# TobiaMarcucci/warm-start-hybrid-mpc

Measured on AMD Instinct MI355X. Metric: QP subproblems/sec, cart-pole-with-walls N=20 synthetic frontier, higher is better.
Workload: dtype f64

## Files before the change

warm-start-hybrid-mpc_amd/csrc/hmpc_device.h:

```cpp
#ifndef HMPC_DEVICE_H
#define HMPC_DEVICE_H

#include <stdint.h>

#include "hmpc.h"

struct SparseStage {
    int m, mg;
    const int *rptr, *rcol;
    const double *rval;
    const int *cptr, *crow;
    const double *cval;
    const int *gptr, *grow;
    const double *gval;
    const double *h;
    const double *scale;
};

#define HMPC_KC_STRIDE 16

struct DevProb {
    int nx, nu, nub, nuc, nz, T, nc, ncL, nT, mreg, Toff, M, Mpad, n, ne, nq, nr, nqT, n_primal, n_dual;
    unsigned mreg_magic;
    int nnz0, nng0;
    SparseStage reg;
    const double *Creg;
    const double *ccv;
    const int *cci;
    int kcol;
    int ngram;
    const double *F_raw, *G_raw, *h_raw, *hT_raw;
    const double *shift_Mmu, *shift_Mrho, *shift_V;
    int *work_counter;
    unsigned *check_flag;
    double *fac_ws;
    int fac_stride;
    int ring;
    int nd, ndp, ns;
    const double *Cdn;
    const int *drow;
    const int *rinfo;
    const double *sval;
    const int *sptr, *srow;
    const int *nrow;
    unsigned nd_magic, nn_magic;
    int split_lds;
    int static_rows;
    const double *Ct, *ht, *sct;
    const double *A, *B, *P, *PT, *Q, *R, *QT;
    const int *ei, *ej;
    double cs;
    double tol, tol_inf;
    int max_iter, lazy, refine;
    int dbg;
    int polish;
    int polish_l1;
    double ptol;
};

struct DevOut {
    double *obj, *dual_obj;
    int32_t *status, *iters;
    double *primal, *dual;
};

struct DevWarm {
    const double *primal, *dual;
    const int32_t *index;
    int32_t *pend;
    int32_t second;
};

static inline size_t hmpc_lds_bytes(const DevProb &p, int kc, int big)
{
    const size_t n = p.n, T = p.T, nx = p.nx, nu = p.nu, nz = p.nz, nub = p.nub, M = p.M;
    size_t d = 0, i = 0, b = 0;
    const size_t nxs = nx * (nx + 1) / 2, lms = nx * nu + nu * (nu - 1) / 2;
    const size_t dir = n + (T + 1) * nx + T * nub, fscr = nz * nz + (kc > 0 ? nz * nz : nx * nz);
    d += dir;
    d += M;
    d += T * nu + (big ? 0 : T * lms + (T + 1) * nxs);
    d += n + T * nx + (T + 1) * nx + n + (T + 1) * nx;
    d += dir + (dir > fscr ? dir : fscr);
    d += (nx + 3) / 4 * 4 + nz + 40;
    d += nx;
    if (big) {
        const size_t nur = (nu + 3) / 4 * 4, nup = (nu + 1 + 3) / 4 * 4, lrows = nz + 1 > nx + nur ? nz + 1 : nx + nur;
        d += ((nx + 1 + 3) / 4 * 4) * lrows + nz * nz + nx * nx;
        d += 2 * (size_t)p.ring * lrows * nup + lms;
    } else {
        d += nx * nz + nz * nz + nx * nx;
    }
    i += 2 + T * nub + 2 * (size_t)p.ne;
    if (!big) {
        i += (p.ne + 1) + p.nng0;
        d += p.mreg + p.nng0;
    }
    if (big) {
    } else if (kc > 0) {
        d += nz * (size_t)kc;
        b += (nz * (size_t)kc + 3) / 4 * 4;
    } else {
        d += 2 * (size_t)p.nnz0;
        i += (p.mreg + 1) + p.nnz0 + (nz + 1) + p.nnz0;
    }
    if (kc == 0 && p.split_lds) {
        d += (size_t)p.ndp * nz + p.mreg;
        i += (size_t)p.ndp + p.mreg + (nz + 1) + p.ns + (p.mreg - p.nd);
    }
    return d * sizeof(double) + i * sizeof(int) + b;
}

#endif
```

warm-start-hybrid-mpc_amd/csrc/hmpc_kernel.hip:

```cpp
#include <hip/hip_runtime.h>
#include <math.h>
#include <stdint.h>
#include <type_traits>

#include "hmpc_device.h"

#define WAVE 64
#define HMPC_REFINE_FROM_IT 12
#define HMPC_POLISH_RHO 1e5
#define HMPC_POLISH_RHO2 1e7
#define HMPC_POLISH_DELTA 1e-10
#define HMPC_RHO_OF(level) ((level) == 1 ? HMPC_POLISH_RHO2 : HMPC_POLISH_RHO)
#define HMPC_POLISH_ITERS 5
#define HMPC_POLISH_ROUNDS 6
#define HMPC_POLISH_ROUNDS_LAST 10
#define HMPC_ESC_MAX 2
#define HMPC_ESC_ITERS 6
#define HMPC_ESC_ENABLED(D) true
#define HMPC_LAM0_ROW 1
#ifndef HMPC_STABLE_DEN
#define HMPC_STABLE_DEN 1
#endif
#ifndef HMPC_PAIR
#define HMPC_PAIR 1
#endif
#ifndef HMPC_NARROW_PANEL
#define HMPC_NARROW_PANEL 1
#endif
#define HMPC_POLISH_ATTEMPTS 3
#define HMPC_RETRY (-1)
#define HMPC_POLISH_ROUNDS_WARM 3
#ifndef HMPC_POLISH_ROUNDS_OWN
#define HMPC_POLISH_ROUNDS_OWN 8
#endif
#define HMPC_POLISH_WARM_BMOVE 0.5
#define HMPC_POLISH_WARM_VMAX 1e-2
#ifndef HMPC_KERNEL_ATTR
#define HMPC_KERNEL_ATTR
#endif
#define DEV __device__ __forceinline__
#ifdef HMPC_NO_FENCE
#define HMPC_FENCE() do { } while (0)
#else
#define HMPC_FENCE() __builtin_amdgcn_sched_barrier(0)
#endif

#ifdef HMPC_STAMPS
#define DBG_SKIP(bit) (p.dbg & (1 << (bit)))
#define STAMP(k) do { long long now_ = clock64(); tacc[k] += now_ - tlast; tlast = clock64(); } while (0)
#define FSTAMP(k) do { long long now_ = clock64(); facc[k] += now_ - flast; flast = clock64(); } while (0)
#define FSTAMP_DECL long long flast = clock64()
static __device__ long long facc_dump[16];
#define FSTAMP_ARGS , long long *facc
#define FSTAMP_PASS , facc
#else
#define DBG_SKIP(bit) false
#define STAMP(k) do { } while (0)
#define FSTAMP(k) do { } while (0)
#define FSTAMP_DECL do { } while (0)
#define FSTAMP_ARGS
#define FSTAMP_PASS
#endif

DEV void lds_barrier()
{
    asm volatile("s_waitcnt lgkmcnt(0)\n\ts_barrier" ::: "memory");
}

DEV double wave_sum(double v)
{
#pragma unroll
    for (int o = 32; o > 0; o >>= 1) v += __shfl_xor(v, o);
    return v;
}
DEV double wave_max(double v)
{
#pragma unroll
    for (int o = 32; o > 0; o >>= 1) v = fmax(v, __shfl_xor(v, o));
    return v;
}
DEV double wave_min(double v)
{
#pragma unroll
    for (int o = 32; o > 0; o >>= 1) v = fmin(v, __shfl_xor(v, o));
    return v;
}

template <class D, int N>
DEV void block_reduce(double (&v)[N], const int (&op)[N], __attribute__((address_space(3))) double *red, int tid)
{
#pragma unroll
    for (int i = 0; i < N; i++) v[i] = op[i] == 0 ? wave_sum(v[i]) : op[i] == 1 ? wave_max(v[i]) : wave_min(v[i]);
    if constexpr (D::kNW > 1) {
        if ((tid & 63) == 0) {
#pragma unroll
            for (int i = 0; i < N; i++) red[(tid >> 6) * N + i] = v[i];
        }
        __syncthreads();
#pragma unroll
        for (int i = 0; i < N; i++) {
            double a = red[i];
#pragma unroll
            for (int w = 1; w < D::kNW; w++) {
                const double b = red[w * N + i];
                a = op[i] == 0 ? a + b : op[i] == 1 ? fmax(a, b) : fmin(a, b);
            }
            v[i] = a;
        }
        __syncthreads();
    }
}
template <class D> DEV double block_sum(double x, __attribute__((address_space(3))) double *red, int tid)
{
    double v[1] = {x};
    const int op[1] = {0};
    block_reduce<D, 1>(v, op, red, tid);
    return v[0];
}
template <class D> DEV double block_max(double x, __attribute__((address_space(3))) double *red, int tid)
{
    double v[1] = {x};
    const int op[1] = {1};
    block_reduce<D, 1>(v, op, red, tid);
    return v[0];
}
template <class D> DEV double block_min(double x, __attribute__((address_space(3))) double *red, int tid)
{
    double v[1] = {x};
    const int op[1] = {2};
    block_reduce<D, 1>(v, op, red, tid);
    return v[0];
}

DEV double bcast(double v, int src)
{
    const int lo = __builtin_amdgcn_readlane(__double2loint(v), src);
    const int hi = __builtin_amdgcn_readlane(__double2hiint(v), src);
    return __hiloint2double(hi, lo);
}

template <class D> DEV double bcast16(double v, int src)
{
    if constexpr (!D::kDpp) return bcast(v, src);
    const long x = __builtin_bit_cast(long, v);
    long r;
    switch (src) {
#define HMPC_DPP_CASE(n) case n: r = __builtin_amdgcn_update_dpp((long)0, x, 0x150 + n, 0xf, 0xf, false); break;
        HMPC_DPP_CASE(0) HMPC_DPP_CASE(1) HMPC_DPP_CASE(2) HMPC_DPP_CASE(3) HMPC_DPP_CASE(4) HMPC_DPP_CASE(5) HMPC_DPP_CASE(6) HMPC_DPP_CASE(7)
        HMPC_DPP_CASE(8) HMPC_DPP_CASE(9) HMPC_DPP_CASE(10) HMPC_DPP_CASE(11) HMPC_DPP_CASE(12) HMPC_DPP_CASE(13) HMPC_DPP_CASE(14)
#undef HMPC_DPP_CASE
    default: r = __builtin_amdgcn_update_dpp((long)0, x, 0x150 + 15, 0xf, 0xf, false); break;
    }
    return __builtin_bit_cast(double, r);
}

DEV double frcp(double b)
{
    double r = __builtin_amdgcn_rcp(b);
    r = fma(fma(-b, r, 1.0), r, r);
    r = fma(fma(-b, r, 1.0), r, r);
    return r;
}

typedef __attribute__((address_space(3))) double ldsd;
typedef __attribute__((address_space(3))) int ldsi;
typedef __attribute__((address_space(3))) unsigned char ldsb;

template <class IP, class DP>
struct Lists {
    IP rptr, rcol, cptr, crow, gptr, grow;
    DP rval, cval, gval, h;
};
typedef Lists<const ldsi *, const ldsd *> ListsL;
typedef Lists<const int *, const double *> ListsG;

struct Lds {
    ldsd *w, *lam, *nuf;
// ... 889 lines not shown
        }
#pragma unroll
        for (int qp = 0; qp < MQ; qp += 2) {
            if (stage && have[qp] && have[qp + 1] && (nx & 3) == 0) {
                const int i0 = trow[qp] + c0, ic0 = i0 < nz ? i0 : nz - 1, jc0 = colq[qp] < nz ? colq[qp] : nz - 1;
                const int i1 = trow[qp + 1] + c0, ic1 = i1 < nz ? i1 : nz - 1, jc1 = colq[qp + 1] < nz ? colq[qp + 1] : nz - 1;
                mfma_d4 acc0 = {gq[qp][0], gq[qp][1], gq[qp][2], gq[qp][3]}, acc1 = {gq[qp + 1][0], gq[qp + 1][1], gq[qp + 1][2], gq[qp + 1][3]};
                mfma_pair_k4<5>(wl, nx, [&](int, int k) { return S.AB[k * AB_STRIDE + ic0]; }, [&](int k, int) { return S.PA[k * nz + jc0]; },
                                [&](int, int k) { return S.AB[k * AB_STRIDE + ic1]; }, [&](int k, int) { return S.PA[k * nz + jc1]; }, acc0, acc1);
#pragma unroll
                for (int r = 0; r < 4; r++) { m[qp][r] = acc0[r]; m[qp + 1][r] = acc1[r]; }
            }
        }
#pragma unroll
        for (int qq = 0; qq < MQ; qq++) {
            if (stage && have[qq]) {
                if (!(have[qq & ~1] && have[qq | 1] && (nx & 3) == 0)) {
                const int i = trow[qq] + c0, ic = i < nz ? i : nz - 1, jc = colq[qq] < nz ? colq[qq] : nz - 1;
                mfma_d4 acc = {gq[qq][0], gq[qq][1], gq[qq][2], gq[qq][3]};
                if ((nx & 3) == 0)
                    acc = mfma_tile_k4<5>(wl, nx, [&](int, int k) { return S.AB[k * AB_STRIDE + ic]; }, [&](int k, int) { return S.PA[k * nz + jc]; }, acc);
                else
                    acc = mfma_tile_batched<5>(wl, nx, [&](int, int k) { return S.AB[k * AB_STRIDE + ic]; },
                                               [&](int k, int) { return S.PA[k * nz + jc]; }, acc);
#pragma unroll
                for (int r = 0; r < 4; r++) m[qq][r] = acc[r];
                }
                if (tcol[qq] + 15 >= nx) {
#pragma unroll
                    for (int r = 0; r < 4; r++) {
                        const int row = row0[qq] + 4 * r, col = colq[qq];
                        ldsd *w = (row < nz && col < nz) ? Mf + row * nz + col : dump;
                        *w = m[qq][r];
                    }
                }
                if (trow[qq] != tcol[qq] && trow[qq] + 15 >= nx) {
#pragma unroll
                    for (int r = 0; r < 4; r++) {
                        const int row = row0[qq] + 4 * r, col = colq[qq];
                        ldsd *w = (row < nz && col < nz) ? Mf + col * nz + row : dump;
                        *w = m[qq][r];
                    }
                }
            }
        }
        if (stage) lds_barrier();
        FSTAMP(1);
        if (!tilew) {
          if (stage) {
            const int i = lane, ic = i < nz ? i : 0, b0 = nx + nuc;
            const int fxv = i < nub ? fx[i < nub ? i : 0] : -1;
            const unsigned long long fm1 = __ballot(fxv >= 0), fone = __ballot(fxv == 1);
            unsigned fixmask = (unsigned)(fm1 << nuc);
            if (i < nz) {
                double g = 0;
                for (int b = 0; b < nub; b++)
                    if ((fone >> b) & 1ull) g += Mf[i * nz + b0 + b];
                S.g[t * nz + i] = g;
            }
            const bool rowfixed = i >= nx && i < nz && ((fixmask >> (i - nx)) & 1u);
            auto panel = [&](auto nc_, int ncols) {
                constexpr int NC = decltype(nc_)::value;
                double a[NC];
#pragma unroll
                for (int k = 0; k < NC; k++) {
                    const double x = Mf[ic * nz + nx + (k < ncols ? k : 0)];
                    const bool pres = rowfixed || ((fixmask >> k) & 1u);
                    a[k] = (k < ncols && i < nz) ? (pres ? (i == nx + k ? 1.0 : 0.0) : x) : 0.0;
                }
                int nuo = __builtin_amdgcn_readfirstlane(ncols);
                unsigned fmask = __builtin_amdgcn_readfirstlane(fixmask);
#pragma unroll
                for (int j = 0; j < NC; j++) {
                    asm volatile("" : "+s"(nuo), "+s"(fmask));
                    if (j < nuo) {
                        if (i < nz) Mf[i * nz + nx + j] = a[j];
                        if ((fmask >> j) & 1u) {
                            if (lane == 0) S.dinv[t * nu + j] = 1.0;
                        } else {
                            const double d = bcast(a[j], nx + j);
                            if (!(d > 0.0)) bad = 1;
                            double rinv = __builtin_amdgcn_rcp(d);
                            rinv = rinv * (2.0 - d * rinv);
                            const bool trailing = i < nx || (i > nx + j && i < nz);
                            const double mval = a[j] * rinv, meff = trailing ? mval : 0.0;
#pragma unroll
                            for (int k = j + 1; k < NC; k++) a[k] -= meff * bcast(a[k], nx + j);
                            if (trailing) Lw[i < nx ? LM_X(nx, nu, i, j) : LM_U(nx, nu, i - nx, j)] = mval;
                            if (lane == 0) S.dinv[t * nu + j] = rinv;
                        }
                    }
                }
            };
            constexpr int NUMC = 8;
            if (HMPC_NARROW_PANEL && nub > 0 && nuc <= NUMC && __popcll(fm1) == nub) {
                panel(std::integral_constant<int, NUMC>(), nuc);
                if (lane < nub) S.dinv[t * nu + nuc + lane] = 1.0;
            } else {
                panel(std::integral_constant<int, NUM>(), nu);
            }
            if (bad && lane == 0) S.flag[0] = 1;
          }
        } else if (t > 0) {
            gram(t - 1);
        }
        if (!stage) continue;
        lds_barrier();
        FSTAMP(3);
#pragma unroll
        for (int qq = 0; qq < MQ; qq++) {
            if (have[qq] && trow[qq] < nx && tcol[qq] < nx) {
                const int i = trow[qq] + c0, ixc = i < nx ? i : nx - 1, k = colq[qq], kc = k < nx ? k : nx - 1;
                mfma_d4 acc = {m[qq][0], m[qq][1], m[qq][2], m[qq][3]};
                acc = mfma_tile_batched<4>(wl, nu, [&](int, int j) { return -Lw[LM_X(nx, nu, ixc, j)]; },
                                           [&](int j, int) { return Mf[kc * nz + nx + j]; }, acc);
#pragma unroll
                for (int r = 0; r < 4; r++) {
                    const int row = row0[qq] + 4 * r, col = colq[qq];
                    if (row < nx && col <= row) {
                        const double v = acc[r];
                        Mf[row * nz + col] = v;
                        Mf[col * nz + row] = v;
                        fac_pr<D>(S)[t * nxs + sym(row, col)] = v;
                    }
                }
            }
        }
        if constexpr (D::kBig)
            for (int e = lane; e < lms; e += D::kNT) Lm[e] = Lw[e];
        lds_barrier();
        FSTAMP(4);
    }
    __syncthreads();
    return (bad || S.flag[0]) ? -1 : 0;
}

template <class D> DEV int factor_reg(const DevProb &p, const Lds &S, int lane FSTAMP_ARGS)
{
    constexpr int NX = D::kNX, NU = D::kNU, NUB = D::kNUB, NUC = NU - NUB, NZ = NX + NU, NE = NZ * (NZ + 1) / 2;
    static_assert(NZ <= 16, "the register recursions broadcast inside one row of 16 lanes");
    constexpr int NXS = NX * (NX + 1) / 2, LMS = LM_STAGE(NX, NU), KG = D::kKC, GH = KG / 2;
    const int T = p.T;
    FSTAMP_DECL;
    LANE_OPAQUE(lane);
    if (lane == 0) S.flag[0] = 0;
    if (D::kNW == 1 || lane < WAVE) {
        const int ng = p.ngram;
        const bool has = lane < ng;
        const int ge = has ? lane : 0;
        const int gi = S.ei[ge], gj = S.ej[ge];
        const int gp0 = S.L0.gptr[ge], glen = has ? S.L0.gptr[ge + 1] - gp0 : 0;
        const double pij = S.P[gi * NZ + gj];
        ldsd *TG = S.Mm + NZ * NZ;
        for (int q = ng + lane; q < NE; q += WAVE) {
            const int i = S.ei[q], j = S.ej[q];
            const double a = S.P[i * NZ + j];
            S.Mm[i * NZ + j] = a;
            S.Mm[j * NZ + i] = a;
        }
        if (S.term_on) {
            const ldsd *Dt = S.e + p.Toff;
            if (p.nT == 0) {
                for (int q = lane; q < NZ * NZ; q += WAVE) TG[q] = 0.0;
            }
            for (int r0 = 0; r0 < p.nT; r0 += WAVE) {
                const int row = r0 + lane;
                const bool ok = row < p.nT;
                const int rc = ok ? row : 0;
                const double dr = ok ? Dt[rc] : 0.0;
                const double *c = p.Ct + (size_t)rc * NZ;
                double cr[NZ];
#pragma unroll
                for (int j = 0; j < NZ; j++) cr[j] = c[j];
#pragma unroll
                for (int i = 0; i < NZ; i++) {
#pragma unroll
                    for (int j = 0; j <= i; j++) {
                        const double a = wave_sum(cr[i] * cr[j] * dr);
                        if (lane == 0) {
                            const double v = (r0 ? TG[i * NZ + j] : 0.0) + a;
                            TG[i * NZ + j] = v;
                            TG[j * NZ + i] = v;
                        }
                    }
                }
            }
        }
        double ABc[NX], pn[NX];
#pragma unroll
        for (int l = 0; l < NX; l++) ABc[l] = lane < NZ ? S.AB[l * NZ + lane] : 0.0;
#pragma unroll
        for (int i = 0; i < NX; i++) pn[i] = lane < NX ? S.PT[i * NX + lane] : 0.0;
        if (lane < NX) {
#pragma unroll
            for (int i = 0; i < NX; i++)
                if (i >= lane) S.Pr[T * NXS + sym(i, lane)] = pn[i];
        }
        int bad = 0;
        for (int t = T - 1; t >= 0; t--) {
            const ldsi *fx = S.fix + t * NUB;
            ldsd *Lm = S.Lm + t * LMS;
            int fxv[NUB];
#pragma unroll
            for (int b = 0; b < NUB; b++) fxv[b] = fx[b];
            double g0 = pij, g1 = 0.0;
            {
                const ldsd *Dt = S.e + t * p.mreg;
#pragma unroll
                for (int hb = 0; hb < KG; hb += GH) {
                    int idx[GH];
                    double gv[GH], dv[GH];
#pragma unroll
                    for (int q = 0; q < GH; q++) {
                        const int qq = gp0 + (hb + q < glen ? hb + q : 0);
                        idx[q] = S.L0.grow[qq];
                        gv[q] = S.L0.gval[qq];
                    }
                    HMPC_FENCE();
#pragma unroll
                    for (int q = 0; q < GH; q++) { HMPC_CHK(idx[q] >= 0 && idx[q] < p.mreg, 2); dv[q] = Dt[idx[q]]; }
                    HMPC_FENCE();
#pragma unroll
                    for (int q = 0; q < GH; q++) {
                        const double term = hb + q < glen ? gv[q] * dv[q] : 0.0;
                        if (q & 1) g1 += term;
                        else g0 += term;
                    }
                }
            }
            if (has) {
                S.Mm[gi * NZ + gj] = g0 + g1;
                S.Mm[gj * NZ + gi] = g0 + g1;
            }
            if (ng > WAVE) {
                const bool has2 = WAVE + lane < ng;
                const int ge2 = has2 ? WAVE + lane : 0;
                const int gi2 = S.ei[ge2], gj2 = S.ej[ge2];
                const int gq0 = S.L0.gptr[ge2], glen2 = has2 ? S.L0.gptr[ge2 + 1] - gq0 : 0;
                const ldsd *Dt = S.e + t * p.mreg;
                double h0 = S.P[gi2 * NZ + gj2], h1 = 0.0;
#pragma unroll
                for (int q = 0; q < KG; q++) {
                    const int qq = gq0 + (q < glen2 ? q : 0);
                    const double term = q < glen2 ? S.L0.gval[qq] * Dt[S.L0.grow[qq]] : 0.0;
                    if (q & 1) h1 += term;
                    else h0 += term;
                }
                if (has2) {
                    S.Mm[gi2 * NZ + gj2] = h0 + h1;
                    S.Mm[gj2 * NZ + gi2] = h0 + h1;
                }
            }
            double y[NX];
#pragma unroll
            for (int i = 0; i < NX; i++) {
                double a = 0.0;
#pragma unroll
                for (int l = 0; l < NX; l++) a += bcast16<D>(pn[l < i ? l : i], l < i ? i : l) * ABc[l];
                y[i] = a;
            }
            double col[NZ];
#pragma unroll
            for (int i = 0; i < NZ; i++) {
                double a = 0.0;
#pragma unroll
                for (int l = 0; l < NX; l++) a += S.AB[l * NZ + i] * y[l];
                col[i] = a;
            }
            FSTAMP(0);
            if (lane < NZ) {
#pragma unroll
                for (int i = 0; i < NZ; i++) col[i] += S.Mm[i * NZ + lane];
                if (S.term_on && t == T - 1) {
#pragma unroll
                    for (int i = 0; i < NZ; i++) col[i] += TG[i * NZ + lane];
                }
            } else {
#pragma unroll
                for (int i = 0; i < NZ; i++) col[i] = 0.0;
            }
            FSTAMP(1);
            int nfixed = 0;
#pragma unroll
            for (int b = 0; b < NUB; b++) nfixed += fxv[b] >= 0;
            if (nfixed) {
                double mbv[NZ];
#pragma unroll
                for (int i = 0; i < NZ; i++) mbv[i] = 0.0;
#pragma unroll
                for (int b = 0; b < NUB; b++)
                    if (fxv[b] == 1) {
#pragma unroll
                        for (int i = 0; i < NZ; i++) mbv[i] += bcast16<D>(col[i], NX + NUC + b);
                    }
                if (lane == 0) {
#pragma unroll
                    for (int i = 0; i < NZ; i++) S.g[t * NZ + i] = mbv[i];
                }
#pragma unroll
                for (int b = 0; b < NUB; b++)
                    if (fxv[b] >= 0) {
                        const int cb = NX + NUC + b;
#pragma unroll
                        for (int i = 0; i < NZ; i++)
                            col[i] = (lane == cb) ? (i == cb ? 1.0 : 0.0) : (i == cb ? 0.0 : col[i]);
                    }
            } else if (lane < NZ) {
                S.g[t * NZ + lane] = 0.0;
            }
            FSTAMP(2);
            double myrow[NU], dinv[NU];
            auto pivot = [&](const int j) {
                const int pj = NX + j;
                const double d = bcast16<D>(col[pj], pj);
                if (!(d > 0.0)) bad = 1;
                double rinv = __builtin_amdgcn_rcp(d);
                rinv = rinv * (2.0 - d * rinv);
                dinv[j] = rinv;
                const double cr = col[pj] * rinv;
                myrow[j] = (lane < NX || lane > pj) ? cr : 0.0;
#pragma unroll
                for (int i = 0; i < NZ; i++) {
                    if (i < NX || i > pj) col[i] -= bcast16<D>(col[i], pj) * cr;
                }
            };
#pragma unroll
            for (int j = 0; j < NUC; j++) pivot(j);
            if ((S.fullfix >> t) & 1ull) {
#pragma unroll
                for (int j = NUC; j < NU; j++) { myrow[j] = 0.0; dinv[j] = 1.0; }
            } else {
#pragma unroll
                for (int j = NUC; j < NU; j++) pivot(j);
            }
            if (lane < NZ) {
                ldsd *row = Lm + (lane < NX ? lane * NU : LM_U(NX, NU, lane - NX, 0));
#pragma unroll
                for (int j = 0; j < NU; j++)
                    if (lane < NX || j < lane - NX) row[j] = myrow[j];
            }
            if (lane < NU) {
                double dv = 1.0;
#pragma unroll
                for (int j = 0; j < NU; j++) dv = (lane == j) ? dinv[j] : dv;
                S.dinv[t * NU + lane] = dv;
            }
            FSTAMP(3);
#pragma unroll
            for (int i = 0; i < NX; i++) pn[i] = col[i];
            if (lane < NX) {
#pragma unroll
                for (int i = 0; i < NX; i++)
                    if (i >= lane) S.Pr[t * NXS + sym(i, lane)] = col[i];
            }
            FSTAMP(4);
        }
        if (lane == 0 && bad) S.flag[0] = 1;
    }
    __syncthreads();
    return S.flag[0] ? -1 : 0;
}

template <class D>
DEV void kkt_sweeps_wave(const DevProb &p, const Lds &S, int lane, bool usex0, const ldsd *csrc, double cs, bool useb, ldsd *dw FSTAMP_ARGS)
{
    FSTAMP_DECL;
    const int nx = D::nx(p), nu = D::nu(p), nz = D::nz(p), T = p.T, nuc = D::nuc(p), nub = D::nub(p);
    const int nxs = nx * (nx + 1) / 2, lms = LM_STAGE(nx, nu);
    const bool w0 = lane < WAVE;
    for (int o = lane; o < T * nx; o += D::kNT) {
        const int t = o / nx, i = o - t * nx;
        double a = 0.0;
        if (csrc) {
            const auto Pn = fac_pr<D>(S) + (t + 1) * nxs;
            int l = 0;
            for (; l + 4 <= nx; l += 4) {
                const double p0 = Pn[sym(i, l)], p1 = Pn[sym(i, l + 1)], p2 = Pn[sym(i, l + 2)], p3 = Pn[sym(i, l + 3)];
                a += p0 * (cs * csrc[t * nx + l]) + p1 * (cs * csrc[t * nx + l + 1]) + p2 * (cs * csrc[t * nx + l + 2]) + p3 * (cs * csrc[t * nx + l + 3]);
            }
            for (; l < nx; l++) a += Pn[sym(i, l)] * (cs * csrc[t * nx + l]);
        }
        S.pv[o] = a;
    }
    double pvr = 0.0;
    double xr = 0.0;
    constexpr int BK = 8;
    auto backward = [&](int t, const ldsd *Lm) {
        const ldsi *fx = S.fix + t * nub;
        const int j = lane;
        const double qv = lane < nx ? pvr + S.pv[t * nx + lane] : 0.0;
        const int jc = j < nz ? j : 0;
        double v = j < nz ? S.g[t * nz + jc] : 0.0, v1 = 0.0;
        for (int l0 = 0; l0 < nx; l0 += BK) {
            double c[BK];
#pragma unroll
            for (int i = 0; i < BK; i++) {
                const int l = l0 + i;
                const double x = S.AB[(l < nx ? l : nx - 1) * AB_STRIDE + jc];
                c[i] = (l < nx && j < nz) ? x : 0.0;
            }
            __builtin_amdgcn_sched_barrier(0);
#pragma unroll
            for (int i = 0; i < BK; i++) {
                const int l = l0 + i;
                const double q = bcast(qv, l < WAVE ? l : WAVE - 1);
                if (i & 1) v1 += c[i] * q;
                else v += c[i] * q;
            }
        }
        v += v1;
        if (j >= nx + nuc && j < nz) {
            const int f = fx[j - nx - nuc];
            if (f >= 0) v = (useb && f == 1) ? -1.0 : 0.0;
        }
        const int rowoff = j < nx ? LM_X(nx, nu, j, 0) : j < nz ? LM_U(nx, nu, j - nx, 0) : 0;
        const int rowlen = j < nx ? nu : j < nz ? j - nx : 0;
        for (int j0 = 0; j0 < nu; j0 += BK) {
            double c[BK];
#pragma unroll
            for (int i = 0; i < BK; i++) {
                const int jj = j0 + i;
                const double x = Lm[rowoff + (jj < rowlen ? jj : 0)];
                c[i] = jj < rowlen ? x : 0.0;
            }
            __builtin_amdgcn_sched_barrier(0);
// ... 1624 lines not shown
        }
        STAMP(6);
        if (!(tau > 0) || !(kap >= 0)) { status = HMPC_NUMERICAL; break; }
        it++;
    }
#ifdef HMPC_STAMPS
    double *tb = trace ? trace - (term_on ? 64 * 8 : 0) + 2 * 64 * 8 : nullptr;
    if (tb && lane == 0)
        for (int k = 0; k < 8; k++) tb[(term_on ? 8 : 0) + k] = (double)tacc[k];
    if (tb && lane == 0 && (term_on == 0 || p.nT == 0))
        for (int k = 0; k < 16; k++) tb[16 + k] = (double)facc[k];
#endif
    iters = it;
    tau_out = tau;
    return status;
}

template <class D> DEV double terminal_violation(const DevProb &p, const Lds &S, int lane, double tau)
{
    double tv = -1e300;
    for (int k = lane; k < p.nT; k += D::kNT) {
        const double a = crow_dot<D>(p, S, p.mreg + k, S.w + (p.T - 1) * D::nz(p)) - p.ht[k] * tau;
        tv = fmax(tv, a / tau);
    }
    return block_max<D>(tv, S.red, lane);
}

template <class D>
DEV void write_record(const DevProb &p, const Lds &S, int lane, int status, double tau, int qp, const DevOut &out)
{
    const int nx = D::nx(p), nu = D::nu(p), nz = D::nz(p), T = p.T, nub = D::nub(p), M = p.M;
    const int nmu = (T - 1) * p.nc + p.ncL;
    const bool inf = status == HMPC_INFEASIBLE;
    double scale;
    if (inf) {
        double big = 0;
        for (int r = lane; r < M; r += D::kNT) big = fmax(big, S.e[r]);
        for (int o = lane; o < (T + 1) * nx; o += D::kNT) big = fmax(big, fabs(S.lam[o]));
        for (int o = lane; o < T * nub; o += D::kNT) big = fmax(big, fabs(S.nuf[o]));
        scale = 1.0 / block_max<D>(big, S.red, lane);
    } else {
        scale = 1.0 / (tau * p.cs);
    }
    double *dual = out.dual ? out.dual + (size_t)qp * p.n_dual : nullptr;
    double *prim = out.primal ? out.primal + (size_t)qp * p.n_primal : nullptr;
    const int o_mu = (T + 1) * nx, o_lb = o_mu + nmu, o_ub = o_lb + T * nub, o_rho = o_ub + T * nub;
    const int o_sig = o_rho + T * p.nq + p.nqT;
    double farkas = 0;
    for (int o = lane; o < (T + 1) * nx; o += D::kNT) {
        const double v = S.lam[o] * scale;
        if (dual) dual[o] = v;
        if (o < nx) farkas -= S.x0[o] * v;
    }
    for (int r = lane; r < M; r += D::kNT) {
        int t, lr;
        row_decode(p, r, t, lr);
        if (lr < p.nc || lr >= p.mreg) {
            const double sc = lr < p.nc ? p.reg.scale[lr] : p.sct[lr - p.mreg];
            const double v = S.e[r] * scale * sc;
            if (dual) dual[o_mu + t * p.nc + (lr < p.nc ? lr : p.nc + (lr - p.mreg))] = v;
            farkas -= (hrow<D>(p, S, lr) / sc) * v;
        }
    }
    for (int o = lane; o < T * nub; o += D::kNT) {
        const int t = o / nub, b = o - t * nub;
        double lo, hi;
        if (S.fix[o] < 0) {
            lo = S.e[t * p.mreg + p.nc + b] * scale;
            hi = S.e[t * p.mreg + p.nc + nub + b] * scale;
            farkas -= hi;
        } else {
            const double v = S.nuf[o] * scale;
            hi = v > 0 ? v : 0.0;
            lo = v < 0 ? -v : 0.0;
            farkas -= S.fix[o] * (hi - lo);
        }
        if (dual) { dual[o_lb + o] = lo; dual[o_ub + o] = hi; }
    }
    farkas = block_sum<D>(farkas, S.red, lane);
    double cost = 0, dq = 0;
    if (inf) {
        if (prim) for (int o = lane; o < p.n_primal; o += D::kNT) prim[o] = __longlong_as_double(0x7ff8000000000000LL);
        if (dual) for (int o = o_rho + lane; o < p.n_dual; o += D::kNT) dual[o] = 0.0;
    } else {
        if (prim) {
            for (int o = lane; o < (T + 1) * nx; o += D::kNT) prim[o] = S.w[(o / nx) * nz + (o % nx)] / tau;
            for (int o = lane; o < T * nu; o += D::kNT) prim[(T + 1) * nx + o] = S.w[(o / nu) * nz + nx + (o % nu)] / tau;
        }
        for (int o = lane; o < T * p.nq + p.nqT; o += D::kNT) {
            const int t = (p.nq > 0 && o / p.nq < T) ? o / p.nq : T;
            const int r = o - t * p.nq;
            const double *QQ = t < T ? p.Q : p.QT;
            double a = 0;
            for (int j = 0; j < nx; j++) a += QQ[r * nx + j] * S.w[t * nz + j];
            a /= tau;
            if (dual) dual[o_rho + o] = 2 * a;
            cost += a * a;
        }
        for (int o = lane; o < T * p.nr; o += D::kNT) {
            const int t = o / p.nr, r = o - t * p.nr;
            double a = 0;
            for (int j = 0; j < nu; j++) a += p.R[r * nu + j] * S.w[t * nz + nx + j];
            a /= tau;
            if (dual) dual[o_sig + o] = 2 * a;
            cost += a * a;
        }
        cost = block_sum<D>(cost, S.red, lane);
        dq = 4.0 * cost;
    }
    if (lane == 0) {
        if (out.obj) out.obj[qp] = inf ? __longlong_as_double(0x7ff0000000000000LL) : cost;
        if (out.dual_obj) out.dual_obj[qp] = inf ? farkas : -0.25 * dq + farkas;
        if (out.status) out.status[qp] = status;
    }
}

template <int NX_, int NU_, int NUB_, int KF, int KB, int KT, int NW, bool WARM = false>
__global__ void __launch_bounds__(NW * WAVE) HMPC_KERNEL_ATTR
hmpc_qp_kernel(const DevProb p_arg, const double *__restrict__ x0g, int x0_stride, const int8_t *__restrict__ fixg, int B,
               const DevOut out, double *__restrict__ rows_ws, double *__restrict__ trace, const int32_t *__restrict__ order, const DevWarm warm)
{
    extern __shared__ __attribute__((aligned(16))) char smem[];
#ifdef HMPC_SIZED
    DevProb p = p_arg;
    HMPC_SIZED(p)
#else
    const DevProb &p = p_arg;
#endif
    constexpr int RS = KF + KB + KT;
#if defined(HMPC_SIZED) && !defined(HMPC_DPP_FEW)
    typedef Dims<NX_, NU_, NUB_, NW, (NX_ > 0 && RS > 0)> D;
#else
    typedef Dims<NX_, NU_, NUB_, NW, (NX_ > 0 && RS > 0 && RS <= 8)> D;
#endif
#ifdef HMPC_SIZED
    static_assert(NX_ <= 0 || RS > 0, "a sized register kernel keeps its row slots");
#else
    static_assert((NX_ > 0) == (RS > 0), "compile-time shapes use the static row map, the generic kernels the lists");
#endif
    typedef typename std::conditional<(NX_ > 0), RowMapS<D, KF, KB, KT>, RowMapL<D>>::type RM;
    const int lane = threadIdx.x;
    const int nx = D::nx(p), nu = D::nu(p), nz = D::nz(p), T = p.T, nub = D::nub(p), M = p.M, n = T * nz + nx, ne = D::ne(p);
    Lds S;
    {
        ldsd *q = (ldsd *)smem;
        auto take = [&](int cnt) { ldsd *r = q; q += cnt; return r; };
        S.w = take(n); S.lam = take((T + 1) * nx); S.nuf = take(T * nub);
        S.e = take(M);
        const int nxs = nx * (nx + 1) / 2;
        S.Lm = take(D::kBig ? 0 : T * LM_STAGE(nx, nu)); S.dinv = take(T * nu); S.Pr = take(D::kBig ? 0 : (T + 1) * nxs);
        S.LmG = p.fac_ws + (size_t)blockIdx.x * p.fac_stride; S.PrG = S.LmG + (size_t)T * LM_STAGE(nx, nu);
        S.rd = take(n); S.rdyn = take(T * nx); S.edyn = take((T + 1) * nx); S.g = take(n); S.pv = take((T + 1) * nx);
        S.w1 = take(n); S.lam1 = take((T + 1) * nx); S.nuf1 = take(T * nub);
        const int dir2 = n + (T + 1) * nx + T * nub, fscr = nz * nz + (D::kKC > 0 ? nz * nz : nx * nz);
        S.w2 = take(dir2 > fscr ? dir2 : fscr); S.lam2 = S.w2 + n; S.nuf2 = S.lam2 + (T + 1) * nx;
        S.Mm = S.w2; S.PA = S.Mm + nz * nz;
        S.q = take((nx + 3) / 4 * 4); S.mv = take(nz); S.red = take(40);
        S.x0 = take(nx);
        S.abst = nz; S.nup = 0; S.lrows = 0;
        int abrows = nx;
        if constexpr (D::kBig) {
            const int nur = (nu + 3) / 4 * 4;
            S.nup = (nu + 1 + 3) / 4 * 4;
            S.lrows = nz + 1 > nx + nur ? nz + 1 : nx + nur;
            S.abst = S.lrows;
            abrows = (nx + 1 + 3) / 4 * 4;
        }
        S.AB = take(abrows * S.abst); S.P = take(nz * nz); S.PT = take(nx * nx);
        constexpr int KC = D::kKC;
        constexpr bool NL = KC > 0 || D::kBig;
        ldsd *h0 = take(D::kBig ? 0 : p.mreg), *rval0 = take(NL ? 0 : p.nnz0), *cval0 = take(KC ? nz * KC : NL ? 0 : p.nnz0);
        ldsd *gval0 = take(D::kBig ? 0 : p.nng0);
        const bool split = KC == 0 && p.split_lds;
        ldsd *cdn0 = take(split ? p.ndp * nz : 0), *sval0 = take(split ? p.mreg : 0);
        S.Ls = take(D::kBig ? 2 * p.ring * S.lrows * S.nup : 0);
        S.Lw = take(D::kBig ? LM_STAGE(nx, nu) : 0);
        if constexpr (D::kBig)
            for (int i = lane; i < 2 * p.ring * S.lrows * S.nup; i += D::kNT) S.Ls[i] = 0.0;
        ldsi *qi = (ldsi *)q;
        auto takei = [&](int cnt) { ldsi *r = qi; qi += cnt; return r; };
        S.flag = takei(2);
        S.fix = takei(T * nub);
        S.ei = takei(ne); S.ej = takei(ne);
        ldsi *rptr0 = takei(NL ? 0 : p.mreg + 1), *rcol0 = takei(NL ? 0 : p.nnz0), *cptr0 = takei(NL ? 0 : nz + 1);
        ldsi *crow0 = takei(NL ? 0 : p.nnz0);
        ldsi *gptr0 = takei(D::kBig ? 0 : ne + 1), *grow0 = takei(D::kBig ? 0 : p.nng0);
        ldsi *drow0 = takei(split ? p.ndp : 0), *rinfo0 = takei(split ? p.mreg : 0), *sptr0 = takei(split ? nz + 1 : 0), *srow0 = takei(split ? p.ns : 0), *nrow0 = takei(split ? p.mreg - p.nd : 0);
        ldsb *cci0 = (ldsb *)qi;
        const SparseStage &g0 = p.reg;
        if constexpr (D::kBig)
            for (int i = lane; i < abrows * S.abst; i += D::kNT) S.AB[i] = 0.0;
        __syncthreads();
        for (int i = lane; i < nx * nz; i += D::kNT) {
            const int l = i / nz, j = i - l * nz;
            S.AB[l * AB_STRIDE + j] = j < nx ? p.A[l * nx + j] : p.B[l * nu + (j - nx)];
        }
        for (int i = lane; i < nz * nz; i += D::kNT) S.P[i] = p.P[i];
        for (int i = lane; i < nx * nx; i += D::kNT) S.PT[i] = p.PT[i];
        if constexpr (!D::kBig)
            for (int i = lane; i < p.mreg; i += D::kNT) h0[i] = g0.h[i];
        if constexpr (D::kBig) {
        } else if constexpr (KC > 0) {
            for (int i = lane; i < nz * KC; i += D::kNT) {
                const int j = i / KC, qq = i - j * KC;
                cval0[i] = p.ccv[j * HMPC_KC_STRIDE + qq];
                cci0[i] = (unsigned char)p.cci[j * HMPC_KC_STRIDE + qq];
            }
        } else {
            for (int i = lane; i < p.nnz0; i += D::kNT) { rval0[i] = g0.rval[i]; cval0[i] = g0.cval[i]; rcol0[i] = g0.rcol[i]; crow0[i] = g0.crow[i]; }
            for (int i = lane; i < p.mreg + 1; i += D::kNT) rptr0[i] = g0.rptr[i];
            for (int i = lane; i < nz + 1; i += D::kNT) cptr0[i] = g0.cptr[i];
        }
        if constexpr (!D::kBig) {
            for (int i = lane; i < p.nng0; i += D::kNT) { gval0[i] = g0.gval[i]; grow0[i] = g0.grow[i]; }
            for (int i = lane; i < ne + 1; i += D::kNT) gptr0[i] = g0.gptr[i];
        }
        for (int i = lane; i < ne; i += D::kNT) { S.ei[i] = p.ei[i]; S.ej[i] = p.ej[i]; }
        S.L0 = ListsL{rptr0, rcol0, cptr0, crow0, gptr0, grow0, rval0, cval0, gval0, h0};
        S.G0 = ListsG{g0.rptr, g0.rcol, g0.cptr, g0.crow, g0.gptr, g0.grow, g0.rval, g0.cval, g0.gval, g0.h};
        S.ccv = cval0;
        S.Cdn = split ? cdn0 : nullptr;
        S.sval = sval0; S.drow = drow0; S.rinfo = rinfo0; S.sptr = sptr0; S.srow = srow0; S.nrow = nrow0;
        if (split) {
            for (int i = lane; i < p.ndp * nz; i += D::kNT) cdn0[i] = p.Cdn[i];
            for (int i = lane; i < p.mreg; i += D::kNT) { sval0[i] = p.sval[i]; rinfo0[i] = p.rinfo[i]; }
            for (int i = lane; i < p.ndp; i += D::kNT) drow0[i] = p.drow[i];
            for (int i = lane; i < nz + 1; i += D::kNT) sptr0[i] = p.sptr[i];
            for (int i = lane; i < p.ns; i += D::kNT) srow0[i] = p.srow[i];
            for (int i = lane; i < p.mreg - p.nd; i += D::kNT) nrow0[i] = p.nrow[i];
        }
        S.cci = cci0;
        S.term_on = 0;
        S.fullfix = 0;
    }
    Rows<RS> R;
    R.bind(rows_ws + (size_t)blockIdx.x * 4 * p.Mpad, p.Mpad);
    RM rm;
    rm.init(p, lane);
    rm.bind(p, S);
    int Bn = B;
    if constexpr (WARM) { if (warm.second) Bn = warm.pend[0]; }
    for (int slot = blockIdx.x, guard = 0; slot < Bn && guard <= Bn; guard++) {
        int qp = order ? order[slot] : slot;
        if constexpr (WARM) { if (warm.second) qp = warm.pend[1 + slot]; }
        __syncthreads();
        for (int o = lane; o < T * nub; o += D::kNT) S.fix[o] = fixg[(size_t)qp * T * nub + o];
        for (int i = lane; i < nx; i += D::kNT) S.x0[i] = x0g[(size_t)qp * x0_stride + i];
        __syncthreads();
        {
            const int st = lane & 63;
            bool all = st < T && nub > 0;
            for (int bq = 0; bq < nub; bq++) all = all && S.fix[(st < T ? st : 0) * nub + bq] >= 0;
            S.fullfix = __ballot(all);
        }
#ifdef HMPC_CHECK
        {
#ifdef HMPC_POISON_FINITE
            const double poison = 1.0;
#else
            const double poison = __longlong_as_double(0x7ff8dead0000beefLL);
#endif
            for (ldsd *q = S.w + lane; q < S.red; q += D::kNT) *q = poison;
            const int nslot = RS > 0 ? RS : p.Mpad / D::kNT;
#pragma unroll
            for (int k = 0; k < nslot; k++) {
#ifndef HMPC_POISON_MASK
#define HMPC_POISON_MASK 15
#endif
                if constexpr (RS > 0) {
                    if (HMPC_POISON_MASK & 1) R.s_[k] = poison;
                    if (HMPC_POISON_MASK & 2) R.zd_[k] = poison;
                    if (HMPC_POISON_MASK & 4) R.dz_[k] = poison;
                    if (HMPC_POISON_MASK & 8) R.prod_[k] = poison;
                }
            }
            __syncthreads();
        }
#endif
        int it1 = 0, it2 = 0, status = HMPC_MAXITER;
        bool polished = false, handed = false, second = false;
        int weak = 0;
        double tau = 1.0;
        double *tr = (trace && qp == 0) ? trace : nullptr;
        const double *wprim = nullptr, *wdual = nullptr;
        if constexpr (WARM) {
            const int wrow = warm.second == 1 ? qp : warm.index ? warm.index[qp] : -1;
            wprim = wrow >= 0 ? warm.primal + (size_t)wrow * p.n_primal : nullptr;
            wdual = wrow >= 0 ? warm.dual + (size_t)wrow * p.n_dual : nullptr;
        }
        const int first = (p.nT > 0 && p.lazy) ? 0 : 1;
        if constexpr (!WARM) {
            for (int term_on = first; term_on < 2; term_on++) {
                int its = 0;
                S.term_on = term_on;
                status = ipm_solve<D, RS, RM, WARM>(p, S, R, rm, lane, term_on, its, tau, polished, weak, handed, tr ? tr + term_on * 64 * 8 : nullptr, wprim, wdual, false);
                if (term_on == 0) it1 = its; else it2 = its;
                if (term_on == 0) {
                    bool done = status == HMPC_INFEASIBLE;
                    if (status == HMPC_OPTIMAL) done = terminal_violation<D>(p, S, lane, tau) < 0.0;
                    if (done) break;
                    if (warm.pend) {
                        if (lane == 0) warm.pend[1 + atomicAdd(warm.pend, 1)] = qp;
                        break;
                    }
                }
            }
        } else {
// ... 224 lines not shown
```

Baseline: 631,400.

## Compute next stage's Gram block one step ahead in double-buffered LDS

Within the backward Riccati factorization, each stage's Gram matrix (P plus constraint outer products) is now computed one stage ahead into an alternating second LDS buffer. The current stage's column is loaded into registers before the next Gram computation starts. This lets the Gram work overlap with the recursion's dependent chain instead of sitting serially on it. In exchange it uses more LDS scratch (an extra nz*nz buffer) and more registers, which could lower occupancy.

New measurement: 635,500 (median of 6 runs). Within noise of the previous version (+0.7%).

```diff
diff --git a/warm-start-hybrid-mpc_amd/csrc/hmpc_device.h b/warm-start-hybrid-mpc_amd/csrc/hmpc_device.h
--- a/warm-start-hybrid-mpc_amd/csrc/hmpc_device.h
+++ b/warm-start-hybrid-mpc_amd/csrc/hmpc_device.h
@@ -76,7 +76,7 @@
     const size_t n = p.n, T = p.T, nx = p.nx, nu = p.nu, nz = p.nz, nub = p.nub, M = p.M;
     size_t d = 0, i = 0, b = 0;
     const size_t nxs = nx * (nx + 1) / 2, lms = nx * nu + nu * (nu - 1) / 2;
-    const size_t dir = n + (T + 1) * nx + T * nub, fscr = nz * nz + (kc > 0 ? nz * nz : nx * nz);
+    const size_t dir = n + (T + 1) * nx + T * nub, fscr = nz * nz + (kc > 0 ? 2 * nz * nz : nx * nz);
     d += dir;
     d += M;
     d += T * nu + (big ? 0 : T * lms + (T + 1) * nxs);
diff --git a/warm-start-hybrid-mpc_amd/csrc/hmpc_kernel.hip b/warm-start-hybrid-mpc_amd/csrc/hmpc_kernel.hip
--- a/warm-start-hybrid-mpc_amd/csrc/hmpc_kernel.hip
+++ b/warm-start-hybrid-mpc_amd/csrc/hmpc_kernel.hip
@@ -23,6 +23,9 @@
 #endif
 #ifndef HMPC_PAIR
 #define HMPC_PAIR 1
+#endif
+#ifndef HMPC_GRAM_AHEAD
+#define HMPC_GRAM_AHEAD 1
 #endif
 #ifndef HMPC_NARROW_PANEL
 #define HMPC_NARROW_PANEL 1
@@ -1218,11 +1221,15 @@
         const int gp0 = S.L0.gptr[ge], glen = has ? S.L0.gptr[ge + 1] - gp0 : 0;
         const double pij = S.P[gi * NZ + gj];
         ldsd *TG = S.Mm + NZ * NZ;
+        auto Mb = [&](const int k) -> ldsd * { return S.Mm + (HMPC_GRAM_AHEAD && (k & 1) ? 2 * NZ * NZ : 0); };
         for (int q = ng + lane; q < NE; q += WAVE) {
             const int i = S.ei[q], j = S.ej[q];
             const double a = S.P[i * NZ + j];
-            S.Mm[i * NZ + j] = a;
-            S.Mm[j * NZ + i] = a;
+#pragma unroll
+            for (int b = 0; b < (HMPC_GRAM_AHEAD ? 2 : 1); b++) {
+                Mb(b)[i * NZ + j] = a;
+                Mb(b)[j * NZ + i] = a;
+            }
         }
         if (S.term_on) {
             const ldsd *Dt = S.e + p.Toff;
@@ -1262,16 +1269,10 @@
             for (int i = 0; i < NX; i++)
                 if (i >= lane) S.Pr[T * NXS + sym(i, lane)] = pn[i];
         }
-        int bad = 0;
-        for (int t = T - 1; t >= 0; t--) {
-            const ldsi *fx = S.fix + t * NUB;
-            ldsd *Lm = S.Lm + t * LMS;
-            int fxv[NUB];
-#pragma unroll
-            for (int b = 0; b < NUB; b++) fxv[b] = fx[b];
+        auto gram = [&](const int tg, ldsd *const Mg) {
             double g0 = pij, g1 = 0.0;
             {
-                const ldsd *Dt = S.e + t * p.mreg;
+                const ldsd *Dt = S.e + tg * p.mreg;
 #pragma unroll
                 for (int hb = 0; hb < KG; hb += GH) {
                     int idx[GH];
@@ -1295,15 +1296,15 @@
                 }
             }
             if (has) {
-                S.Mm[gi * NZ + gj] = g0 + g1;
-                S.Mm[gj * NZ + gi] = g0 + g1;
+                Mg[gi * NZ + gj] = g0 + g1;
+                Mg[gj * NZ + gi] = g0 + g1;
             }
             if (ng > WAVE) {
                 const bool has2 = WAVE + lane < ng;
                 const int ge2 = has2 ? WAVE + lane : 0;
                 const int gi2 = S.ei[ge2], gj2 = S.ej[ge2];
                 const int gq0 = S.L0.gptr[ge2], glen2 = has2 ? S.L0.gptr[ge2 + 1] - gq0 : 0;
-                const ldsd *Dt = S.e + t * p.mreg;
+                const ldsd *Dt = S.e + tg * p.mreg;
                 double h0 = S.P[gi2 * NZ + gj2], h1 = 0.0;
 #pragma unroll
                 for (int q = 0; q < KG; q++) {
@@ -1313,10 +1314,30 @@
                     else h0 += term;
                 }
                 if (has2) {
-                    S.Mm[gi2 * NZ + gj2] = h0 + h1;
-                    S.Mm[gj2 * NZ + gi2] = h0 + h1;
-                }
-            }
+                    Mg[gi2 * NZ + gj2] = h0 + h1;
+                    Mg[gj2 * NZ + gi2] = h0 + h1;
+                }
+            }
+        };
+#if HMPC_GRAM_AHEAD
+        gram(T - 1, Mb(T - 1));
+#endif
+        int bad = 0;
+        for (int t = T - 1; t >= 0; t--) {
+            const ldsi *fx = S.fix + t * NUB;
+            ldsd *Lm = S.Lm + t * LMS;
+            int fxv[NUB];
+#pragma unroll
+            for (int b = 0; b < NUB; b++) fxv[b] = fx[b];
+            ldsd *const Mt = Mb(t);
+#if HMPC_GRAM_AHEAD
+            double m0[NZ];
+#pragma unroll
+            for (int i = 0; i < NZ; i++) m0[i] = Mt[i * NZ + (lane < NZ ? lane : 0)];
+            if (t > 0) gram(t - 1, Mb(t - 1));
+#else
+            gram(t, Mt);
+#endif
             double y[NX];
 #pragma unroll
             for (int i = 0; i < NX; i++) {
@@ -1336,7 +1357,11 @@
             FSTAMP(0);
             if (lane < NZ) {
 #pragma unroll
-                for (int i = 0; i < NZ; i++) col[i] += S.Mm[i * NZ + lane];
+#if HMPC_GRAM_AHEAD
+                for (int i = 0; i < NZ; i++) col[i] += m0[i];
+#else
+                for (int i = 0; i < NZ; i++) col[i] += Mt[i * NZ + lane];
+#endif
                 if (S.term_on && t == T - 1) {
 #pragma unroll
                     for (int i = 0; i < NZ; i++) col[i] += TG[i * NZ + lane];
@@ -3267,7 +3292,7 @@
         S.LmG = p.fac_ws + (size_t)blockIdx.x * p.fac_stride; S.PrG = S.LmG + (size_t)T * LM_STAGE(nx, nu);
         S.rd = take(n); S.rdyn = take(T * nx); S.edyn = take((T + 1) * nx); S.g = take(n); S.pv = take((T + 1) * nx);
         S.w1 = take(n); S.lam1 = take((T + 1) * nx); S.nuf1 = take(T * nub);
-        const int dir2 = n + (T + 1) * nx + T * nub, fscr = nz * nz + (D::kKC > 0 ? nz * nz : nx * nz);
+        const int dir2 = n + (T + 1) * nx + T * nub, fscr = nz * nz + (D::kKC > 0 ? 2 * nz * nz : nx * nz);
         S.w2 = take(dir2 > fscr ? dir2 : fscr); S.lam2 = S.w2 + n; S.nuf2 = S.lam2 + (T + 1) * nx;
         S.Mm = S.w2; S.PA = S.Mm + nz * nz;
         S.q = take((nx + 3) / 4 * 4); S.mv = take(nz); S.red = take(40);
```
